# robertknight/ocrs

Measured on AMD Instinct MI355X. Metric: pages/sec end-to-end (1024x1024), higher is better.
Workload: dtype f32

## Files before the change

### include/ocrs_amd.h

```cpp
#ifndef OCRS_AMD_H
#define OCRS_AMD_H

#include <stddef.h>
#include <stdint.h>

#if defined(__GNUC__)
#define OCRS_API __attribute__((visibility("default")))
#else
#define OCRS_API
#endif

#ifdef __cplusplus
extern "C" {
#endif

typedef enum ocrs_status {
    OCRS_OK = 0,
    OCRS_ERR_INVALID_ARGUMENT = 1,
    OCRS_ERR_MODEL_NOT_LOADED = 2,
    OCRS_ERR_MODEL_DIMS = 3,
    OCRS_ERR_RUN_FAILED = 4,
    OCRS_ERR_WRONG_OUTPUT = 5,
    OCRS_ERR_IMAGE_SOURCE = 6,
    OCRS_ERR_DEVICE = 7,
// ... 23 lines not shown

OCRS_API ocrs_status ocrs_mask_component_rects(const uint8_t* masks, size_t n, int h, int w, float expand, float min_area,
                                               int max_comp, int64_t arena, int32_t* n_roots, int32_t* overflow, float* rects,
                                               uint8_t* valid);

OCRS_API ocrs_status ocrs_gru_tile_plan(const int32_t* lengths_desc, size_t n_lines, int hidden, int32_t* n_clusters, int32_t* waves,
                                        int16_t* tiles);

OCRS_API ocrs_status ocrs_coalescer_selftest(int n_threads, int requests_per_thread, int max_active, int max_pages,
                                             long window_us, int fail_every, uint64_t out[5]);

OCRS_API ocrs_status ocrs_stream_plan_selftest(int budget, const int32_t* ops, size_t n_ops, int32_t* out);

OCRS_API ocrs_status ocrs_conv_rows_selftest(const float* w, size_t n_w, const float* bias, size_t n_bias, int relu, int y0, int h,
                                             int cin, int32_t out[6]);

OCRS_API ocrs_status ocrs_set_option(const char* name, long value);
OCRS_API ocrs_status ocrs_option_name(int index, const char** name);

OCRS_API ocrs_status ocrs_device_pool_stats(int device, uint64_t out[12]);
OCRS_API ocrs_status ocrs_device_pool_configure(int device, uint64_t device_cached_cap_bytes, uint64_t pinned_cached_cap_bytes);
OCRS_API ocrs_status ocrs_device_pool_trim(int device);

typedef enum { OCRS_ISOLATION_AUTO = 0, OCRS_ISOLATION_NONE = 1 } ocrs_isolation;
OCRS_API ocrs_status ocrs_device_set_isolation(int device, ocrs_isolation policy);
OCRS_API ocrs_status ocrs_device_isolation(int device, int out[3]);

typedef struct ocrs_model ocrs_model;

OCRS_API ocrs_status ocrs_model_load_file(const char* path, ocrs_model** out);
// ... 428 lines not shown
```

### ocrs_amd/_lib.py

```python
import ctypes as C
import os

_HERE = os.path.dirname(os.path.abspath(__file__))
LIB_PATH = os.environ.get("OCRS_AMD_LIB") or os.path.join(_HERE, "libocrs_amd.so")

OCRS_OK = 0
STATUS_NAMES = {
    0: "OK", 1: "INVALID_ARGUMENT", 2: "MODEL_NOT_LOADED", 3: "MODEL_DIMS", 4: "RUN_FAILED", 5: "WRONG_OUTPUT",
    6: "IMAGE_SOURCE", 7: "DEVICE", 8: "IO", 9: "CAPACITY",
}

RUN_FN = C.CFUNCTYPE(C.c_int, C.c_void_p, C.POINTER(C.c_float), C.POINTER(C.c_int64), C.POINTER(C.POINTER(C.c_float)),
                     C.POINTER(C.c_int64), C.POINTER(C.c_int))


class EngineParams(C.Structure):
    _fields_ = [("detection_model", C.c_void_p), ("recognition_model", C.c_void_p), ("debug", C.c_int),
                ("decode_method", C.c_int), ("beam_width", C.c_uint32), ("alphabet", C.c_char_p),
                ("allowed_chars", C.c_char_p), ("numerics", C.c_int), ("coalesce", C.c_int), ("coalesce_pages", C.c_int),
                ("coalesce_window_us", C.c_int), ("layout_threads", C.c_int), ("rec_max_pixels", C.c_int64)]


class GroupParams(C.Structure):
    _fields_ = [("detection_model", C.c_void_p), ("detection_model_len", C.c_size_t), ("recognition_model", C.c_void_p),
# ... 24 lines not shown
    "ocrs_last_error", "ocrs_buffer_free", "ocrs_device_count", "ocrs_set_device", "ocrs_set_option", "ocrs_ctc_beam_search", "ocrs_model_load_file",
    "ocrs_model_load_bytes", "ocrs_model_from_callback", "ocrs_model_input_shape", "ocrs_model_run",
    "ocrs_model_flops", "ocrs_model_free", "ocrs_engine_new", "ocrs_engine_free", "ocrs_image_source_check_bytes",
    "ocrs_engine_prepare_input", "ocrs_engine_prepare_input_device", "ocrs_page_free", "ocrs_page_dims",
    "ocrs_page_image", "ocrs_engine_detect_words", "ocrs_engine_detect_words_batch",
    "ocrs_engine_detect_text_pixels", "ocrs_engine_detection_threshold", "ocrs_engine_find_text_lines",
    "ocrs_engine_find_text_lines_batch",
    "ocrs_engine_recognize_text", "ocrs_engine_recognize_text_batch", "ocrs_engine_recognize_tokens",
    "ocrs_engine_prepare_recognition_input", "ocrs_text_item_rotated_rect", "ocrs_rotated_rect_corners", "ocrs_engine_get_text", "ocrs_device_malloc", "ocrs_device_free",
    "ocrs_device_upload", "ocrs_device_synchronize", "ocrs_device_measure_peaks", "ocrs_engine_enable_timing", "ocrs_stage_count",
    "ocrs_stage_name", "ocrs_engine_stage_times", "ocrs_kernel_class_count", "ocrs_kernel_class_name",
    "ocrs_engine_kernel_stats", "ocrs_engine_set_kernel_timing_mask", "ocrs_gru_tile_plan", "ocrs_host_malloc", "ocrs_host_free", "ocrs_engine_prepare_input_batch",
    "ocrs_get_device", "ocrs_model_load_file_on_device", "ocrs_model_load_bytes_on_device", "ocrs_model_device", "ocrs_engine_device",
    "ocrs_engine_group_new", "ocrs_engine_group_free", "ocrs_engine_group_size", "ocrs_engine_group_member", "ocrs_group_deal",
    "ocrs_group_prepare_input_batch", "ocrs_group_prepare_input_device_batch", "ocrs_group_detect_words_batch",
    "ocrs_group_recognize_text_batch", "ocrs_group_gather", "ocrs_group_final_gather", "ocrs_group_worker_threads", "ocrs_group_last_gather", "ocrs_device_malloc_on", "ocrs_engine_coalesce_stats", "ocrs_coalescer_selftest", "ocrs_stream_plan_selftest", "ocrs_conv_rows_selftest", "ocrs_engine_kernel_mfma_flops", "ocrs_engine_prepare_input_jpeg", "ocrs_jpeg_decode_rgb", "ocrs_jpeg_info", "ocrs_jpeg_coefficients",
    "ocrs_group_member_stats", "ocrs_numa_parse_cpulist", "ocrs_numa_bind_selftest", "ocrs_engine_recognize_logits", "ocrs_engine_set_option", "ocrs_engine_get_option", "ocrs_option_name", "ocrs_device_pool_stats", "ocrs_device_pool_configure", "ocrs_device_pool_trim",
    "ocrs_device_set_isolation", "ocrs_device_isolation", "ocrs_group_set_replay", "ocrs_abi_version",
    "ocrs_engine_recognize_text_scored", "ocrs_engine_recognize_text_batch_scored", "ocrs_ctc_beam_search_scored",
    "ocrs_engine_run_recognition_ops", "ocrs_ctc_decode_packed", "ocrs_mask_component_rects",
    "ocrs_engine_detect_words_scored", "ocrs_engine_detect_words_batch_scored", "ocrs_group_detect_words_batch_scored",
    "ocrs_engine_find_text_lines_indexed", "ocrs_engine_find_text_lines_batch_indexed",
    "ocrs_detection_tile_plan", "ocrs_engine_detect_words_tiled", "ocrs_engine_detect_words_batch_tiled",
    "ocrs_engine_detect_text_pixels_tiled", "ocrs_group_detect_words_batch_tiled",
    "ocrs_line_frame", "ocrs_line_char_boxes", "ocrs_engine_prepare_recognition_input_rectified",
    "ocrs_engine_recognize_text_rectified", "ocrs_engine_recognize_text_batch_rectified",
    "ocrs_group_recognize_text_batch_rectified", "ocrs_engine_recognize_tokens_rectified",
    "ocrs_engine_rotate_page", "ocrs_engine_rotate_pages", "ocrs_unrotate_rects", "ocrs_unrotate_chars",
    "ocrs_orientation_vote", "ocrs_engine_detect_orientation", "ocrs_engine_page_from_grey",
    "ocrs_engine_resize_page", "ocrs_engine_resize_pages", "ocrs_work_size", "ocrs_rescale_rects",
    "ocrs_engine_detect_words_at", "ocrs_engine_detect_words_batch_at",
# ... 303 lines not shown
```

### ocrs_amd/csrc/abi.cpp

```cpp
#include <cstdio>
#include <fstream>
#include <thread>

#include <atomic>
#include "abi_util.hpp"
#include "coalesce_selftest.hpp"
#include "conv_rows.hpp"
#include "engine.hpp"
#include "host_pool.hpp"
#include "jpeg.hpp"
#include "kernels.hpp"
#include "page_ops.hpp"

using namespace ocrs;
using namespace ocrs::geom;

using namespace ocrs::abi;

extern "C" {

const char* ocrs_last_error(void) { return last_error().c_str(); }

void ocrs_buffer_free(void* p) { free(p); }

// ... 61 lines not shown

ocrs_status ocrs_conv_rows_selftest(const float* w, size_t n_w, const float* bias, size_t n_bias, int relu, int y0, int h, int cin,
                                    int32_t out[6]) {
    return guarded([&] {
        if (!out || (n_w > 0 && !w) || (n_bias > 0 && !bias) || h < kConvRowsPatchH || h % kConvRowsPatchH != 0 || y0 < 0 || y0 >= h ||
            y0 % kConvRowsPatchH != 0 || cin < 2 * kConvRowsChunk || cin % (2 * kConvRowsChunk) != 0)
            fail(OCRS_ERR_INVALID_ARGUMENT, "bad argument");
        out[0] = conv_rows_skip_exact(w, n_w, bias, n_bias, relu != 0) ? 1 : 0;
        const RowPhases ph = conv_row_phases(y0, h, cin, out[0] != 0);
        out[1] = ph.c_top;
        out[2] = ph.c_bot;
        for (int phase = 0; phase < 3; phase++) {
            const int c = 3 * phase * (cin / kConvRowsChunk);
            out[3 + phase] = c < ph.c_top ? 0 : c >= ph.c_bot ? kConvRowsPatchH - 1 : -1;
        }
    });
}

namespace {

void beam_search_hook(const float* logp, int t, int c, uint32_t width, int impl, std::vector<uint32_t>* l,
                      std::vector<uint32_t>* p, double* score, std::vector<float>* step_logp) {
    if (impl == 2 && t > 0) {
        DeviceScope bind(-1);
        if (!k::ctc_beam_supported(c, (int)width)) fail(OCRS_ERR_CAPACITY, "beam search on the GPU supports up to 128 classes and width 128");
        Workspace ws;
        std::vector<int32_t> meta(1 + t + 1);
        meta[0] = t;
        for (int i = 0; i <= t; i++) meta[1 + i] = i;
        int32_t* d_meta = ws.alloc_n<int32_t>(meta.size());
// ... 1066 lines not shown
```

### ocrs_amd/csrc/common.cpp

```cpp
#include "common.hpp"

#include <chrono>
#include <climits>
#include <cstdint>
#include <cstdlib>
#include <cstring>

#include <algorithm>
#include <atomic>
#include <condition_variable>
#include <deque>
#include <system_error>

namespace ocrs {

static thread_local std::string g_last_error;

void set_last_error(const std::string& msg) { g_last_error = msg; }
const std::string& last_error() { return g_last_error; }

namespace {
std::atomic<int> g_default_device{0};
thread_local DeviceContext* t_ctx = nullptr;
constexpr int kMaxDevices = 64;
// ... 430 lines not shown
const OptRange kOptRanges[OPT_COUNT] = {
    {0, 1, {}}, {0, 1, {}}, {0, 1, {}}, {0, 2, {}}, {0, 1, {8, 14, 32}}, {0, 1, {8, 14, 20, 32}}, {0, 1, {}}, {0, 1, {}}, {0, 1, {}}, {0, 1, {}},
    {1, 1024, {}}, {LanePlan::kMinBudget, LanePlan::kMaxBudget, {}},
    {0, 2, {}}, {0, 64, {}}, {1, 4096, {}}, {0, 10000000, {}}, {0, 4096, {}}, {0, INT64_MAX, {}},
};
bool in_range(int i, long v) {
    const OptRange& r = kOptRanges[i];
    if (i == OPT_STREAM_BUDGET) return LanePlan::valid_budget(v);
    if (v >= r.lo && v <= r.hi) return true;
    for (long a : r.also) if (a && v == a) return true;
    return false;
}
const char* const kRetired[] = {"det_heavy", "det_tail", "gru_waves", "gru_background", "gru_scatter", "gru_gates_pack", "conv_occupancy",
                                "gx_heavy", "gemm_nfast", "conv_a_lds", "gru_heavy", "heavy_priority", "det_mfma"};
std::atomic<long> g_opts[OPT_COUNT];
std::once_flag g_opts_once;
void init_options() {
    for (int i = 0; i < OPT_COUNT; i++) {
        const char* e = kOptDefs[i].env ? getenv(kOptDefs[i].env) : nullptr;
        const long v = e && *e ? strtol(e, nullptr, 10) : kOptDefs[i].def;
        g_opts[i].store(in_range(i, v) ? v : kOptDefs[i].def);
    }
}
int find_option(const char* name, int count = OPT_PUBLIC_COUNT) {
    for (int i = 0; i < count; i++)
        if (name && i != OPT_NUMERICS && strcmp(name, kOptDefs[i].name) == 0) return i;
    return -1;
}
thread_local const Tuning* t_tuning = nullptr;
}
// ... 2 lines not shown
TuningScope::~TuningScope() { t_tuning = prev_; }
const Tuning* current_tuning() { return t_tuning; }

long process_option(Option o) {
    std::call_once(g_opts_once, init_options);
    return g_opts[o].load(std::memory_order_relaxed);
}

long option_long(Option o) {
    if (t_tuning) return __atomic_load_n(&t_tuning->v[o], __ATOMIC_RELAXED);
    std::call_once(g_opts_once, init_options);
    return g_opts[o].load(std::memory_order_relaxed);
}
int option(Option o) { return (int)option_long(o); }
int conv_rows_setting() { return t_tuning ? (int)__atomic_load_n(&t_tuning->conv_rows, __ATOMIC_RELAXED) : (int)kConvRowsDefault; }

Tuning default_tuning() {
    std::call_once(g_opts_once, init_options);
    Tuning t;
    for (int i = 0; i < OPT_COUNT; i++) t.v[i] = g_opts[i].load(std::memory_order_relaxed);
    t.conv_rows = kConvRowsDefault;
    return t;
}

const char* option_name(int i) { return i >= 0 && i < OPT_PUBLIC_COUNT ? kOptDefs[i].name : nullptr; }

int set_option(const char* name, long value) {
    std::call_once(g_opts_once, init_options);
    const int i = find_option(name);
    if (i < 0) {
        for (const char* r : kRetired) if (name && strcmp(name, r) == 0) return 0;
        return 1;
    }
    if (!in_range(i, value)) return 2;
    if (i == OPT_STREAM_BUDGET && value != g_opts[i].load() && any_device_has_calls_in_flight()) return 3;
    g_opts[i].store(value);
    return 0;
}

int set_option(Tuning& t, const char* name, long value) {
    if (name && strcmp(name, "conv_rows") == 0) {
        if (value < 0 || value > 2) return 2;
        __atomic_store_n(&t.conv_rows, value, __ATOMIC_RELAXED);
        return 0;
    }
    const int i = find_option(name, OPT_COUNT);
    if (i < 0) return 1;
    if (i == OPT_STREAM_BUDGET) return 4;
    if (!in_range(i, value)) return 2;
    __atomic_store_n(&t.v[i], value, __ATOMIC_RELAXED);
    return 0;
}

bool get_option(const Tuning& t, const char* name, long* value) {
    if (name && strcmp(name, "conv_rows") == 0) {
        *value = __atomic_load_n(&t.conv_rows, __ATOMIC_RELAXED);
        return true;
    }
    const int i = name && strcmp(name, "numerics") == 0 ? (int)OPT_NUMERICS : find_option(name, OPT_COUNT);
    if (i < 0) return false;
    *value = __atomic_load_n(&t.v[i], __ATOMIC_RELAXED);
    return true;
}

static hipEvent_t take_lease_event(DeviceContext* c) {
    {
        std::lock_guard<std::mutex> g(c->stream_mu);
        if (!c->lease_events.empty()) {
            hipEvent_t e = c->lease_events.back();
            c->lease_events.pop_back();
            return e;
// ... 139 lines not shown
```

### ocrs_amd/csrc/common.hpp

```cpp
#pragma once
#include <atomic>
#include <hip/hip_runtime.h>

#include <cstdarg>
#include <cstdint>
#include <cstdio>
#include <cstdlib>
#include <chrono>
#include <condition_variable>
#include <cstring>
#include <map>
#include <mutex>
#include <stdexcept>
#include <string>
#include <thread>
#include <vector>

#include "../../include/ocrs_amd.h"
#include "stream_plan.hpp"

namespace ocrs {

struct Error : std::runtime_error {
    ocrs_status status;
// ... 116 lines not shown
    DeviceContext* prev_;
    int restore_ = -1;
};

inline DevicePool& pool() { return ctx().pool; }
inline HostPool& host_pool() { return ctx().host_pool; }
inline hipStream_t heavy_stream() { return ctx().heavy_stream(); }

enum Option { OPT_GRU_MODE = 0, OPT_GRU_GATES, OPT_GRU_LOCAL, OPT_DET_FUSE, OPT_DET_STREAM, OPT_DET_ROWS, OPT_CCL_QUAD,
              OPT_CONV12_FUSE, OPT_CONV_FLAT, OPT_BEAM_GPU, OPT_DET_TILE_BATCH, OPT_STREAM_BUDGET, OPT_PUBLIC_COUNT,
              OPT_NUMERICS = OPT_PUBLIC_COUNT,
              OPT_COALESCE, OPT_COALESCE_PAGES, OPT_COALESCE_WINDOW_US,
              OPT_LAYOUT_THREADS, OPT_REC_MAX_PIXELS,
              OPT_COUNT };
constexpr long kConvRowsDefault = 2;
struct Tuning { long v[OPT_COUNT]; long conv_rows; };
int conv_rows_setting();
Tuning default_tuning();
int set_option(const char* name, long value);
int set_option(Tuning& t, const char* name, long value);
bool get_option(const Tuning& t, const char* name, long* value);
const char* option_name(int i);
class TuningScope {
  public:
    explicit TuningScope(const Tuning* t);
    ~TuningScope();
    TuningScope(const TuningScope&) = delete;
    TuningScope& operator=(const TuningScope&) = delete;
  private:
    const Tuning* prev_;
};
const Tuning* current_tuning();
// ... 204 lines not shown
```

### ocrs_amd/csrc/conv_rows.hpp

```cpp
#pragma once
#include <cmath>
#include <cstddef>
#include <cstring>

namespace ocrs {

constexpr int kConvRowsChunk = 16;
constexpr int kConvRowsPatchH = 4;

inline bool conv_rows_skip_exact(const float* w, size_t n_w, const float* bias, size_t n_bias, bool relu) {
    for (size_t i = 0; i < n_w; i++)
        if (!std::isfinite(w[i])) return false;
    if (relu) return true;
    for (size_t i = 0; i < n_bias; i++) {
        unsigned u;
        memcpy(&u, &bias[i], 4);
        if (u == 0x80000000u) return false;
    }
    return true;
}

struct RowPhases { int c_top, c_bot; };
constexpr RowPhases conv_row_phases(int y0, int H, int cin, bool skip) {
    const int per_tap = cin / kConvRowsChunk;
// ... 5 lines not shown
```

### ocrs_amd/csrc/kernels.hpp

```cpp
#pragma once
#include <vector>
#include <hip/hip_runtime.h>

#include <cstdint>

namespace ocrs {
namespace jpeg { struct Coefficients; }
namespace k {

void prepare_image(const void* d_pixels, bool is_u8, bool chans_last, int h, int w, int chans, float* d_out,
                   hipStream_t s);
struct PrepareTable {
    enum { kPages = 32 };
    const void* src[kPages];
    float* dst[kPages];
};
void prepare_image_batch(const void* const* d_pixels, float* const* d_out, int n, bool is_u8, bool chans_last, int h, int w,
                         int chans, hipStream_t s);
void resize_pages_to_model(const float* const* d_src_ptrs, int n, int sh, int sw, int vh, int vw, float* d_dst,
                           int dh, int dw, hipStream_t s);
bool resize_threshold(const float* d_prob, int n, int mh, int mw, int sh, int sw, float thr, uint8_t* d_mask,
                      float* d_map, int h, int w, hipStream_t s, int32_t* d_labels = nullptr, int32_t* d_zero_a = nullptr,
                      int32_t* d_zero_b = nullptr);
void threshold_only(const float* d_prob, float thr, uint8_t* d_mask, int64_t count, hipStream_t s);
// ... 68 lines not shown
    float* y;
    float* ypool;
    int n, h, w, h1, w1;
    int relu_d1, relu_p1, relu_d2, relu_p2, sigmoid;
    int tiles_x, tiles_y;
    const float* tape = nullptr;
    int tape_len = 0;
    const float* rtape = nullptr;
    int rtape_len = 0;
};
struct StreamWeights {
    const float *wt, *bt, *wd1, *bd1, *wp1, *bp1, *wd2, *bd2, *wp2, *bp2, *wf, *bf;
};
bool double_conv_fused(const DoubleConvArgs& a, int cs, int cx, int cmid, int cout, bool pool, bool final_conv,
                       bool launch, hipStream_t s, bool* on_mfma = nullptr, int* path = nullptr);
bool double_conv_stream(const DoubleConvArgs& a, int cs, int cx, int cmid, int cout, bool pool, bool final_conv, bool launch, hipStream_t s,
                        const StreamWeights* hw = nullptr, std::vector<float>* tape_out = nullptr, int* tape_len = nullptr);
bool double_conv_rows(const DoubleConvArgs& a, int cs, int cx, int cmid, int cout, bool pool, bool final_conv, bool launch, hipStream_t s,
                      const StreamWeights* hw = nullptr, std::vector<float>* tape_out = nullptr, int* tape_len = nullptr);
bool double_conv_rows_takes(const DoubleConvArgs& a, int cx);
void maxpool(const float* x, int n, int h, int w, int c, int kh, int kw, float* y, hipStream_t s);
void avgpool(const float* x, int n, int h, int w, int c, int kh, int kw, float* y, hipStream_t s);
void padcat(const float* skip, int n, int sh, int sw, int cs, const float* x, int h, int w, int cx, float* y,
            hipStream_t s);
void sigmoid(const float* x, float* y, int64_t count, hipStream_t s);
void conv1x1_cout1(const float* x, int64_t pixels, int cin, const float* wt, const float* bias, int relu, int do_sigmoid,
                   float* y, hipStream_t s);
void to_seq(const float* x, int n, int w, int c, float* y, hipStream_t s);
void gru_gates(const float* gx, const float* gh, float* h, float* y, int T, int N, int H, int step, hipStream_t s);
bool log_softmax_argmax(const float* logits, int64_t rows, int c, const uint8_t* d_excluded ,
// ... 283 lines not shown
```

### ocrs_amd/csrc/kernels_det.hip

```cpp
#include "common.hpp"
#include "kernels.hpp"
#include "spec_math.hpp"

namespace ocrs {
namespace k {

namespace {

typedef float f32x4 __attribute__((ext_vector_type(4)));

__device__ __forceinline__ int floor_div2(int v) { return v >> 1; }

template <int CS_, int CX_, int CMID_, int COUT_, int TH_, int TW_, bool POOL_, bool FINAL_>
struct McCfg {
    static constexpr int NT = 512;
    static constexpr int CS = CS_, CX = CX_, CMID = CMID_, COUT = COUT_, TH = TH_, TW = TW_;
    static constexpr bool POOL = POOL_, FINAL = FINAL_, DEC = CX_ > 0;
    static constexpr int CU = DEC ? CS_ : 0;
    static constexpr int CIN = CS + CU;
    static constexpr bool ONE = CIN == 1;
    static constexpr int P = TW_ >= 32 ? 4 : 2;
    static constexpr int SA = ONE ? 1 : CIN + 4, SD1 = ONE ? 1 : CIN + 4, SC = CMID + 4, SD2 = CMID + 4, SE = COUT + 4, SX = CX + 4;
    static constexpr int R0H = TH + 4, R0W = TW + 4, R1H = TH + 2, R1W = TW + 2;
    static constexpr int LH = (TH + 4) / 2 + 1, LW = (TW + 4) / 2 + 1;
    static constexpr int NPIX0 = R0H * R0W, NPIX1 = R1H * R1W, NPIX2 = TH * TW;
    static constexpr int A_FLOATS = NPIX0 * SA, C_FLOATS = NPIX1 * SC;
    static constexpr int X_FLOATS = DEC ? LH * LW * SX : 0, D1_FLOATS = ONE ? 0 : NPIX1 * SD1, D2_FLOATS = NPIX2 * SD2;
    static constexpr int E_FLOATS = POOL ? NPIX2 * SE : 0;
    static constexpr int max3(int x, int y, int z) { return (x > y ? x : y) > z ? (x > y ? x : y) : z; }
    static constexpr int U_RAW = ONE ? max3(A_FLOATS, D2_FLOATS, 0) : max3(A_FLOATS, C_FLOATS, E_FLOATS);
    static constexpr int V_RAW = ONE ? max3(C_FLOATS, E_FLOATS, 0) : max3(X_FLOATS, D1_FLOATS, D2_FLOATS);
    static constexpr int U_FLOATS = (U_RAW + 3) / 4 * 4 + 64, V_FLOATS = (V_RAW + 3) / 4 * 4 + 64;
    static constexpr int W_FLOATS = 10 * CIN + 10 * CMID;
    static constexpr size_t LDS_BYTES = (size_t)(U_FLOATS + V_FLOATS + W_FLOATS) * sizeof(float);
};

template <int K> __device__ __forceinline__ constexpr int ch_pos(int c) { return (c & 3) * (K / 4) + (c >> 2); }
template <int K> __device__ __forceinline__ constexpr int ch_of(int n) { return (n % (K / 4)) * 4 + n / (K / 4); }

template <int K, int P, int S_IN, int S_OUT>
__device__ __forceinline__ void dw_stage(const float* __restrict__ src, int srcw, float* __restrict__ dst, int rows, int cols,
                                         const float* __restrict__ sw, bool relu, int tid, int nt) {
    constexpr int NB = K / 4;
    const int ns = (cols + P - 1) / P;
    const int items = rows * ns * NB;
    for (int it = tid; it < items; it += nt) {
        const int blk = it % NB;
        const int t2 = it / NB;
        const int strip = t2 % ns, r = t2 / ns;
        const int x0 = strip * P;
        f32x4 acc[P];
        const f32x4 bias = *reinterpret_cast<const f32x4*>(sw + 9 * K + 4 * blk);
#pragma unroll
        for (int j = 0; j < P; j++) acc[j] = bias;
#pragma unroll
        for (int dy = 0; dy < 3; dy++) {
            f32x4 row[P + 2];
#pragma unroll
            for (int j = 0; j < P + 2; j++) {
                const int xx = x0 + j < srcw ? x0 + j : srcw - 1;
                row[j] = *reinterpret_cast<const f32x4*>(src + ((r + dy) * srcw + xx) * S_IN + 4 * blk);
            }
#pragma unroll
            for (int dx = 0; dx < 3; dx++) {
                const f32x4 wv = *reinterpret_cast<const f32x4*>(sw + (dy * 3 + dx) * K + 4 * blk);
#pragma unroll
                for (int j = 0; j < P; j++) {
#pragma unroll
                    for (int e = 0; e < 4; e++) acc[j][e] = fmaf(row[j + dx][e], wv[e], acc[j][e]);
                }
            }
        }
#pragma unroll
        for (int j = 0; j < P; j++) {
            if (x0 + j < cols) {
                f32x4 v = acc[j];
// ... 12 lines not shown
    if constexpr (KS == 1) {
        b[0] = p[0];
    } else if constexpr (KS == 2) {
        const float2 v = *reinterpret_cast<const float2*>(p);
        b[0] = v.x; b[1] = v.y;
    } else {
#pragma unroll
        for (int q = 0; q < KS / 4; q++) {
            const f32x4 v = *reinterpret_cast<const f32x4*>(p + 4 * q);
            b[4 * q] = v[0]; b[4 * q + 1] = v[1]; b[4 * q + 2] = v[2]; b[4 * q + 3] = v[3];
        }
    }
}

template <class Cfg>
__global__ void __launch_bounds__(Cfg::NT)
double_conv_mfma_kernel(DoubleConvArgs a) {
    constexpr int NT = Cfg::NT, NW = Cfg::NT / 64;
    constexpr int CS = Cfg::CS, CX = Cfg::CX, CU = Cfg::CU, CIN = Cfg::CIN, CMID = Cfg::CMID, COUT = Cfg::COUT;
    constexpr int TH = Cfg::TH, TW = Cfg::TW, SA = Cfg::SA, SD1 = Cfg::SD1, SC = Cfg::SC, SD2 = Cfg::SD2, SE = Cfg::SE, SX = Cfg::SX;
    constexpr int R0H = Cfg::R0H, R0W = Cfg::R0W, R1H = Cfg::R1H, R1W = Cfg::R1W, LH = Cfg::LH, LW = Cfg::LW;
    constexpr int NPIX0 = Cfg::NPIX0, NPIX1 = Cfg::NPIX1, NPIX2 = Cfg::NPIX2, P = Cfg::P;
    extern __shared__ __attribute__((aligned(16))) float lds[];
    float* sU = lds;
    float* sV = lds + Cfg::U_FLOATS;
    float* sW1 = sV + Cfg::V_FLOATS;
    float* sW2 = sW1 + 10 * CIN;
    const int tid = threadIdx.x;
    const int lane = tid & 63, wave = tid >> 6;
    const int i16 = lane & 15, kq = lane >> 4;
    const int nblk = gridDim.x;
// ... 13 lines not shown
    for (int i = tid; i < 10 * CMID; i += NT) {
        const int t = i / CMID, n = i - t * CMID;
        const int c = ch_of<CMID>(n);
        sW2[i] = t < 9 ? a.wd2[t * CMID + c] : a.bd2[c];
    }

    float* sA = sU;
    const float* __restrict__ skip = a.skip + (int64_t)img * h * w * CS;
    if constexpr (Cfg::ONE) {
        for (int p = tid; p < NPIX0; p += NT) {
            const int gy = Y0 - 2 + p / R0W, gx = X0 - 2 + p % R0W;
            float v = 0.f;
            if ((unsigned)gy < (unsigned)h && (unsigned)gx < (unsigned)w) v = skip[(int64_t)gy * w + gx];
            sA[p] = v;
        }
    } else {
        constexpr int Q = CS / 4;
        for (int i = tid; i < NPIX0 * Q; i += NT) {
            const int p = i / Q, c4 = i - p * Q;
            const int gy = Y0 - 2 + p / R0W, gx = X0 - 2 + p % R0W;
            f32x4 v = {0.f, 0.f, 0.f, 0.f};
            if ((unsigned)gy < (unsigned)h && (unsigned)gx < (unsigned)w)
                v = *reinterpret_cast<const f32x4*>(skip + ((int64_t)gy * w + gx) * CS + c4 * 4);
#pragma unroll
            for (int e = 0; e < 4; e++) sA[p * SA + ch_pos<CIN>(c4 * 4 + e)] = v[e];
        }
    }
    if constexpr (Cfg::DEC) {
        float* sX = sV;
        const int pyo = (h - 2 * a.h1) / 2, pxo = (w - 2 * a.w1) / 2;
        const int ly0 = floor_div2(Y0 - 2 - pyo), lx0 = floor_div2(X0 - 2 - pxo);
        const float* __restrict__ x1 = a.x1 + (int64_t)img * a.h1 * a.w1 * CX;
        constexpr int QX = CX / 4, NLOW = LH * LW;
        for (int i = tid; i < NLOW * QX; i += NT) {
            const int p = i / QX, c4 = i - p * QX;
            const int ly = ly0 + p / LW, lx = lx0 + p % LW;
            f32x4 v = {0.f, 0.f, 0.f, 0.f};
            if ((unsigned)ly < (unsigned)a.h1 && (unsigned)lx < (unsigned)a.w1)
                v = *reinterpret_cast<const f32x4*>(x1 + ((int64_t)ly * a.w1 + lx) * CX + c4 * 4);
#pragma unroll
            for (int e = 0; e < 4; e++) sX[p * SX + ch_pos<CX>(c4 * 4 + e)] = v[e];
        }
        for (int i = tid; i < NPIX0 * CU; i += NT) {
            const int p = i / CU, c = i - p * CU;
            sA[p * SA + ch_pos<CIN>(CS + c)] = 0.f;
        }
        constexpr int KSX = CX / 4, NGT = (4 * CU) / 16;
        float at[NGT][KSX];
        f32x4 biast[NGT];
#pragma unroll
        for (int g = 0; g < NGT; g++) {
            const int n = 16 * g + i16, q = n / CU, co = n % CU;
#pragma unroll
            for (int s4 = 0; s4 < KSX; s4++) at[g][s4] = a.wt[((size_t)q * CX + 4 * s4 + kq) * CU + co];
#pragma unroll
            for (int r = 0; r < 4; r++) biast[g][r] = a.bt[(16 * g + 4 * kq + r) % CU];
        }
        __syncthreads();
        for (int pg = wave; pg * 16 < NLOW; pg += NW) {
            const int p = pg * 16 + i16;
            const int pc = p < NLOW ? p : NLOW - 1;
            float b[KSX];
            load_b<KSX>(sX + pc * SX + kq * KSX, b);
            const int ly = ly0 + pc / LW, lx = lx0 + pc % LW;
            const bool src_ok = p < NLOW && (unsigned)ly < (unsigned)a.h1 && (unsigned)lx < (unsigned)a.w1;
#pragma unroll
            for (int g = 0; g < NGT; g++) {
                f32x4 acc = biast[g];
#pragma unroll
                for (int s4 = 0; s4 < KSX; s4++) acc = __builtin_amdgcn_mfma_f32_16x16x4f32(at[g][s4], b[s4], acc, 0, 0, 0);
                const int n0 = 16 * g + 4 * kq;
                const int q = n0 / CU, co0 = n0 % CU;
                const int gy = 2 * ly + (q >> 1) + pyo, gx = 2 * lx + (q & 1) + pxo;
                const int ry = gy - (Y0 - 2), rx = gx - (X0 - 2);
                if (src_ok && (unsigned)ry < (unsigned)R0H && (unsigned)rx < (unsigned)R0W && (unsigned)gy < (unsigned)h &&
                    (unsigned)gx < (unsigned)w) {
#pragma unroll
                    for (int r = 0; r < 4; r++) sA[(ry * R0W + rx) * SA + ch_pos<CIN>(CS + co0 + r)] = acc[r];
                }
            }
        }
    }
    __syncthreads();

    float* sC = sU;
    if constexpr (Cfg::ONE) {
        float* sCt = sV;
        for (int p = tid; p < NPIX1; p += NT) {
            const int ry = p / R1W, rx = p - ry * R1W;
            const int gy = Y0 - 1 + ry, gx = X0 - 1 + rx;
            float* dst = &sCt[p * SC];
            if ((unsigned)gy >= (unsigned)h || (unsigned)gx >= (unsigned)w) {
#pragma unroll
// ... 3 lines not shown
            float d = sW1[9];
#pragma unroll
            for (int t = 0; t < 9; t++) d = fmaf(sA[(ry + t / 3) * R0W + rx + t % 3], sW1[t], d);
            if (a.relu_d1) d = d > 0.f ? d : 0.f;
#pragma unroll
            for (int c = 0; c < CMID; c++) {
                float o = fmaf(d, a.wp1[c], a.bp1[c]);
                if (a.relu_p1) o = o > 0.f ? o : 0.f;
                dst[ch_pos<CMID>(c)] = o;
            }
        }
        __syncthreads();
        sC = sCt;
    } else {
        float* sD1 = sV;
        dw_stage<CIN, P, SA, SD1>(sA, R0W, sD1, R1H, R1W, sW1, a.relu_d1 != 0, tid, NT);
        constexpr int KS = CIN / 4, NG = (CMID + 15) / 16;
        float aw[NG][KS];
        f32x4 bias1[NG];
#pragma unroll
        for (int g = 0; g < NG; g++) {
            const int n = 16 * g + i16;
            const int co = n < CMID ? ch_of<CMID>(n) : 0;
#pragma unroll
            for (int s4 = 0; s4 < KS; s4++) aw[g][s4] = n < CMID ? a.wp1[(4 * s4 + kq) * CMID + co] : 0.f;
#pragma unroll
            for (int r = 0; r < 4; r++) {
                const int nr = 16 * g + 4 * kq + r;
                bias1[g][r] = nr < CMID ? a.bp1[ch_of<CMID>(nr)] : 0.f;
            }
        }
// ... 123 lines not shown

bool double_conv_fused(const DoubleConvArgs& a, int cs, int cx, int cmid, int cout, bool pool, bool final_conv,
                       bool launch, hipStream_t s, bool* on_mfma, int* path) {
    if (path) *path = 0;
    if (option(OPT_DET_ROWS) >= 1 && ((!launch && a.n == 0) || a.rtape) && double_conv_rows_takes(a, cx) &&
        double_conv_rows(a, cs, cx, cmid, cout, pool, final_conv, launch, s)) {
        if (on_mfma) *on_mfma = true;
        if (path) *path = 2;
        return true;
    }
    if (option(OPT_DET_STREAM) >= 1 && ((!launch && a.n == 0) || a.tape) && double_conv_stream(a, cs, cx, cmid, cout, pool, final_conv, launch, s)) {
        if (on_mfma) *on_mfma = false;
        if (path) *path = 1;
        return true;
    }
#define OCRS_DC(CS, CX, CM, CO, TH, TW, P, F)                                                   \
    if (cs == CS && cx == CX && cmid == CM && cout == CO && pool == P && final_conv == F) {      \
        if (on_mfma) *on_mfma = true;                                                            \
        if (launch) launch_mc<McCfg<CS, CX, CM, CO, TH, TW, P, F>>(a, s);                        \
        return true;                                                                             \
    }
    OCRS_DC(1, 0, 8, 8, 16, 32, true, false)
    OCRS_DC(8, 0, 16, 16, 8, 32, true, false)
    OCRS_DC(16, 0, 32, 32, 8, 16, true, false)
    OCRS_DC(32, 0, 32, 32, 8, 16, true, false)
    OCRS_DC(8, 16, 8, 8, 8, 32, false, true)
    OCRS_DC(8, 16, 8, 8, 8, 32, false, false)
    OCRS_DC(16, 32, 16, 16, 8, 16, false, false)
    OCRS_DC(32, 32, 32, 32, 8, 16, false, false)
    OCRS_DC(32, 64, 32, 32, 8, 16, false, false)
#undef OCRS_DC
    return false;
}

}
}
```

### ocrs_amd/csrc/kernels_rec.hip

```cpp
#include <algorithm>
#include <type_traits>

#include "common.hpp"
#include "conv_rows.hpp"
#include "kernels.hpp"
#include "split_mfma.hpp"

namespace ocrs {
namespace k {

typedef float f32x16 __attribute__((ext_vector_type(16)));
typedef unsigned u32x4 __attribute__((ext_vector_type(4)));
typedef float f32x4 __attribute__((ext_vector_type(4)));
typedef float f32x2 __attribute__((ext_vector_type(2)));
typedef unsigned u32x2 __attribute__((ext_vector_type(2)));
typedef __bf16 bf16x8 __attribute__((ext_vector_type(8)));
typedef __bf16 bf16x2 __attribute__((ext_vector_type(2)));

__device__ __forceinline__ int xcd_remap(int b, int nwg) {
    const int xcd = b & 7, q = nwg >> 3, r = nwg & 7;
    return (xcd < r ? xcd * (q + 1) : r * (q + 1) + (xcd - r) * q) + (b >> 3);
}

__device__ __forceinline__ int find_group(const int32_t* __restrict__ toff, int G, int tile) {
// ... 184 lines not shown
void avgpool_to_seq_ragged(const float* x, const RaggedView& in, const RaggedView& seq, int c, const int32_t* d_pos,
                           const int32_t* d_off, float* y, hipStream_t s) {
    if (seq.ntiles256 <= 0) return;
    hipLaunchKernelGGL(avgpool_to_seq_ragged_kernel, dim3(seq.ntiles256), dim3(256), 0, s, x, in, seq, c, d_pos, d_off, y);
}

void to_seq_packed_ragged(const float* x, const RaggedView& in, int c, const int32_t* d_pos, const int32_t* d_off,
                          float* y, hipStream_t s) {
    if (in.ntiles256 <= 0) return;
    hipLaunchKernelGGL(to_seq_packed_ragged_kernel, dim3(in.ntiles256), dim3(256), 0, s, x, in, c, d_pos, d_off, y);
}

constexpr int RG_BM = 128, RG_BK = 16, RG_LDA = RG_BM + 1;
constexpr int CONV_WAVES = 4;
static_assert(RG_BK == kConvRowsChunk && RG_BM / 32 == kConvRowsPatchH, "conv_rows.hpp describes this kernel's K loop");
template <int BN, int TW, int PH, int PW, int ROWS, bool FLAT, int SPLIT = 0>
__global__ void __launch_bounds__(256, SPLIT == 3 ? 2 : SPLIT == 2 ? 3 : CONV_WAVES)
conv3x3_ragged_kernel(const float* __restrict__ X, RaggedView rv, int cin, const float* __restrict__ Bw,
                      const float* __restrict__ bias, int cout, int relu, float* __restrict__ Y,
                      const int64_t* __restrict__ out_poff, int skip) {
    extern __shared__ __attribute__((aligned(16))) float lds[];
    constexpr int NTW = BN / 64;
    constexpr int TH = RG_BM / TW;
    static_assert(TW == 32 || TW == 16, "patch width");
    static_assert(!ROWS || (SPLIT == 0 && BN == 128 && TW == 32), "row-owning waves: exact, 128 columns, 4 x 32 patches");
    static_assert(!SPLIT || (BN == 128 && RG_BK == 16), "split mode: 128-column blocks, 16-deep chunks");
    constexpr int NP = SPLIT ? SPLIT : 1;
    constexpr int SP_PLANE = split::PLANE;
    float* As = lds;
    float* Bs = lds + (SPLIT ? 2 * NP * SP_PLANE : 2 * RG_BK * RG_LDA);
// ... 805 lines not shown
        rv.toff2d_flat = rv_in.toff2d_flat_32; rv.ntiles2d_flat = rv_in.ntiles2d_flat_32;
        rv.toff2d_flat2 = rv_in.toff2d_flat2_32; rv.ntiles2d_flat2 = rv_in.ntiles2d_flat2_32;
        rv.max_tile_px_ = rv_in.max_tile_px32_;
    }
    if (rv.tw != 32 && rv.tw != 16) return false;
    if (rv.H % (RG_BM / rv.tw) != 0) return false;
    const bool flat = option(OPT_CONV_FLAT) != 0 && rv.min_w >= 11 &&
                      rv.max_tile_px_ * std::max(cin, cout) * (int64_t)sizeof(float) < (int64_t)1 << 30;
    if (!flat && (int64_t)rv.H * rv.max_w * cin * (int64_t)sizeof(float) >= (int64_t)1 << 30) return false;
    const int ntiles = flat ? (pw == 2 ? rv.ntiles2d_flat2 : rv.ntiles2d_flat) : rv.ntiles2d;
    if (ntiles <= 0) return true;
    const bool n64 = cout <= 64;
    const int numerics = option(OPT_NUMERICS);
    const bool split = wsplit && !n64 && (cout % 128) == 0 && (cin % 64) == 0 && numerics != 0;
    const size_t lds = split ? split::lds_bytes(numerics == 2 ? 2 : 3)
                             : (size_t)(2 * RG_BK * RG_LDA + 2 * RG_BK * (n64 ? 64 : 128)) * sizeof(float);
    const dim3 grid(ntiles, (cout + (n64 ? 63 : 127)) / (n64 ? 64 : 128));
#define OCRS_LAUNCH_SPLIT(TW_, PH_, PW_, FLAT_, NP_, SLOT_)                                                              \
    if (flat == FLAT_ && (numerics == 2 ? 2 : 3) == NP_) {                                                              \
        allow_dynamic_lds(reinterpret_cast<const void*>(&conv3x3_ragged_kernel<128, TW_, PH_, PW_, 0, FLAT_, NP_>), ok_[SLOT_]);   \
        hipLaunchKernelGGL((conv3x3_ragged_kernel<128, TW_, PH_, PW_, 0, FLAT_, NP_>), grid, dim3(256), lds, s, x, rv, cin, ws_, bias, \
                           cout, relu, y, out.poff, 0);                                                                 \
    }
#define OCRS_LAUNCH_CONV(BN_, TW_, PH_, PW_)                                                                            \
    do {                                                                                                                \
        if (split && BN_ == 128) {                                                                                      \
            const float* ws_ = reinterpret_cast<const float*>(wsplit);                                                  \
            static std::atomic<uint64_t> ok_[4] = {};                                                                    \
            OCRS_LAUNCH_SPLIT(TW_, PH_, PW_, true, 3, 0) OCRS_LAUNCH_SPLIT(TW_, PH_, PW_, false, 3, 1)                     \
            OCRS_LAUNCH_SPLIT(TW_, PH_, PW_, true, 2, 2) OCRS_LAUNCH_SPLIT(TW_, PH_, PW_, false, 2, 3)                     \
        } else if (flat) hipLaunchKernelGGL((conv3x3_ragged_kernel<BN_, TW_, PH_, PW_, 0, true>), grid, dim3(256), lds, s, x, rv, \
// ... 36 lines not shown
```

Before: 288.1.

## Add lean 256-thread detection double-conv variants sized to co-reside with conv blocks

Adds a 'lean' configuration of the fused detection double-conv MFMA kernel that uses 256 threads, smaller tiles, and a two-phase staged load of skip and upsampled channels. Its LDS footprint is capped so it fits beside three resident ragged-conv blocks, so detection can overlap with recognition convs on the same CU. Upsample weights are reloaded per group instead of held in registers when they would be too large. The variant is on by default for batches larger than 8 and can be selected through a new det_lean option. It trades per-block throughput for higher occupancy and co-residency.

Result: no change. 287.5 (-0.2%).

```diff
diff --git a/include/ocrs_amd.h b/include/ocrs_amd.h
--- a/include/ocrs_amd.h
+++ b/include/ocrs_amd.h
@@ -61,6 +61,9 @@
 
 OCRS_API ocrs_status ocrs_conv_rows_selftest(const float* w, size_t n_w, const float* bias, size_t n_bias, int relu, int y0, int h,
                                              int cin, int32_t out[6]);
+
+OCRS_API ocrs_status ocrs_det_block_query(int cs, int cx, int cmid, int cout, int pool, int final_conv, int n, int h, int w,
+                                          int h1, int w1, int tapes, int32_t out[3]);
 
 OCRS_API ocrs_status ocrs_set_option(const char* name, long value);
 OCRS_API ocrs_status ocrs_option_name(int index, const char** name);
diff --git a/ocrs_amd/_lib.py b/ocrs_amd/_lib.py
--- a/ocrs_amd/_lib.py
+++ b/ocrs_amd/_lib.py
@@ -62,7 +62,7 @@
     "ocrs_get_device", "ocrs_model_load_file_on_device", "ocrs_model_load_bytes_on_device", "ocrs_model_device", "ocrs_engine_device",
     "ocrs_engine_group_new", "ocrs_engine_group_free", "ocrs_engine_group_size", "ocrs_engine_group_member", "ocrs_group_deal",
     "ocrs_group_prepare_input_batch", "ocrs_group_prepare_input_device_batch", "ocrs_group_detect_words_batch",
-    "ocrs_group_recognize_text_batch", "ocrs_group_gather", "ocrs_group_final_gather", "ocrs_group_worker_threads", "ocrs_group_last_gather", "ocrs_device_malloc_on", "ocrs_engine_coalesce_stats", "ocrs_coalescer_selftest", "ocrs_stream_plan_selftest", "ocrs_conv_rows_selftest", "ocrs_engine_kernel_mfma_flops", "ocrs_engine_prepare_input_jpeg", "ocrs_jpeg_decode_rgb", "ocrs_jpeg_info", "ocrs_jpeg_coefficients",
+    "ocrs_group_recognize_text_batch", "ocrs_group_gather", "ocrs_group_final_gather", "ocrs_group_worker_threads", "ocrs_group_last_gather", "ocrs_device_malloc_on", "ocrs_engine_coalesce_stats", "ocrs_coalescer_selftest", "ocrs_stream_plan_selftest", "ocrs_conv_rows_selftest", "ocrs_det_block_query","ocrs_engine_kernel_mfma_flops", "ocrs_engine_prepare_input_jpeg", "ocrs_jpeg_decode_rgb", "ocrs_jpeg_info", "ocrs_jpeg_coefficients",
     "ocrs_group_member_stats", "ocrs_numa_parse_cpulist", "ocrs_numa_bind_selftest", "ocrs_engine_recognize_logits", "ocrs_engine_set_option", "ocrs_engine_get_option", "ocrs_option_name", "ocrs_device_pool_stats", "ocrs_device_pool_configure", "ocrs_device_pool_trim",
     "ocrs_device_set_isolation", "ocrs_device_isolation", "ocrs_group_set_replay", "ocrs_abi_version",
     "ocrs_engine_recognize_text_scored", "ocrs_engine_recognize_text_batch_scored", "ocrs_ctc_beam_search_scored",
diff --git a/ocrs_amd/csrc/abi.cpp b/ocrs_amd/csrc/abi.cpp
--- a/ocrs_amd/csrc/abi.cpp
+++ b/ocrs_amd/csrc/abi.cpp
@@ -99,6 +99,22 @@
             const int c = 3 * phase * (cin / kConvRowsChunk);
             out[3 + phase] = c < ph.c_top ? 0 : c >= ph.c_bot ? kConvRowsPatchH - 1 : -1;
         }
+    });
+}
+
+ocrs_status ocrs_det_block_query(int cs, int cx, int cmid, int cout, int pool, int final_conv, int n, int h, int w, int h1, int w1,
+                                 int tapes, int32_t out[3]) {
+    return guarded([&] {
+        if (!out || n < 0 || h < 1 || w < 1 || h1 < 0 || w1 < 0) fail(OCRS_ERR_INVALID_ARGUMENT, "bad argument");
+        static const float dummy = 0.f;
+        k::DoubleConvArgs a{};
+        a.n = n; a.h = h; a.w = w; a.h1 = h1; a.w1 = w1;
+        if (tapes) { a.tape = &dummy; a.rtape = &dummy; }
+        bool on_mfma = false;
+        int path = 0;
+        out[0] = k::double_conv_fused(a, cs, cx, cmid, cout, pool != 0, final_conv != 0, false, nullptr, &on_mfma, &path) ? 1 : 0;
+        out[1] = out[0] ? path : -1;
+        out[2] = det_lean_setting();
     });
 }
 
diff --git a/ocrs_amd/csrc/common.cpp b/ocrs_amd/csrc/common.cpp
--- a/ocrs_amd/csrc/common.cpp
+++ b/ocrs_amd/csrc/common.cpp
@@ -468,6 +468,8 @@
 const char* const kRetired[] = {"det_heavy", "det_tail", "gru_waves", "gru_background", "gru_scatter", "gru_gates_pack", "conv_occupancy",
                                 "gx_heavy", "gemm_nfast", "conv_a_lds", "gru_heavy", "heavy_priority", "det_mfma"};
 std::atomic<long> g_opts[OPT_COUNT];
+std::atomic<long> g_det_lean{kDetLeanDefault};
+bool is_det_lean(const char* name) { return name && strcmp(name, "det_lean") == 0; }
 std::once_flag g_opts_once;
 void init_options() {
     for (int i = 0; i < OPT_COUNT; i++) {
@@ -500,12 +502,16 @@
 }
 int option(Option o) { return (int)option_long(o); }
 int conv_rows_setting() { return t_tuning ? (int)__atomic_load_n(&t_tuning->conv_rows, __ATOMIC_RELAXED) : (int)kConvRowsDefault; }
+int det_lean_setting() {
+    return (int)(t_tuning ? __atomic_load_n(&t_tuning->det_lean, __ATOMIC_RELAXED) : g_det_lean.load(std::memory_order_relaxed));
+}
 
 Tuning default_tuning() {
     std::call_once(g_opts_once, init_options);
     Tuning t;
     for (int i = 0; i < OPT_COUNT; i++) t.v[i] = g_opts[i].load(std::memory_order_relaxed);
     t.conv_rows = kConvRowsDefault;
+    t.det_lean = g_det_lean.load(std::memory_order_relaxed);
     return t;
 }
 
@@ -513,6 +519,11 @@
 
 int set_option(const char* name, long value) {
     std::call_once(g_opts_once, init_options);
+    if (is_det_lean(name)) {
+        if (value < 0 || value > 2) return 2;
+        g_det_lean.store(value);
+        return 0;
+    }
     const int i = find_option(name);
     if (i < 0) {
         for (const char* r : kRetired) if (name && strcmp(name, r) == 0) return 0;
@@ -528,6 +539,11 @@
     if (name && strcmp(name, "conv_rows") == 0) {
         if (value < 0 || value > 2) return 2;
         __atomic_store_n(&t.conv_rows, value, __ATOMIC_RELAXED);
+        return 0;
+    }
+    if (is_det_lean(name)) {
+        if (value < 0 || value > 2) return 2;
+        __atomic_store_n(&t.det_lean, value, __ATOMIC_RELAXED);
         return 0;
     }
     const int i = find_option(name, OPT_COUNT);
@@ -541,6 +557,10 @@
 bool get_option(const Tuning& t, const char* name, long* value) {
     if (name && strcmp(name, "conv_rows") == 0) {
         *value = __atomic_load_n(&t.conv_rows, __ATOMIC_RELAXED);
+        return true;
+    }
+    if (is_det_lean(name)) {
+        *value = __atomic_load_n(&t.det_lean, __ATOMIC_RELAXED);
         return true;
     }
     const int i = name && strcmp(name, "numerics") == 0 ? (int)OPT_NUMERICS : find_option(name, OPT_COUNT);
diff --git a/ocrs_amd/csrc/common.hpp b/ocrs_amd/csrc/common.hpp
--- a/ocrs_amd/csrc/common.hpp
+++ b/ocrs_amd/csrc/common.hpp
@@ -154,8 +154,10 @@
               OPT_LAYOUT_THREADS, OPT_REC_MAX_PIXELS,
               OPT_COUNT };
 constexpr long kConvRowsDefault = 2;
-struct Tuning { long v[OPT_COUNT]; long conv_rows; };
+constexpr long kDetLeanDefault = 1;
+struct Tuning { long v[OPT_COUNT]; long conv_rows; long det_lean; };
 int conv_rows_setting();
+int det_lean_setting();
 Tuning default_tuning();
 int set_option(const char* name, long value);
 int set_option(Tuning& t, const char* name, long value);
diff --git a/ocrs_amd/csrc/conv_rows.hpp b/ocrs_amd/csrc/conv_rows.hpp
--- a/ocrs_amd/csrc/conv_rows.hpp
+++ b/ocrs_amd/csrc/conv_rows.hpp
@@ -7,6 +7,7 @@
 
 constexpr int kConvRowsChunk = 16;
 constexpr int kConvRowsPatchH = 4;
+constexpr size_t kConvRaggedLdsBytes = (size_t)(2 * kConvRowsChunk * (128 + 1) + 2 * kConvRowsChunk * 128) * sizeof(float);
 
 inline bool conv_rows_skip_exact(const float* w, size_t n_w, const float* bias, size_t n_bias, bool relu) {
     for (size_t i = 0; i < n_w; i++)
diff --git a/ocrs_amd/csrc/kernels.hpp b/ocrs_amd/csrc/kernels.hpp
--- a/ocrs_amd/csrc/kernels.hpp
+++ b/ocrs_amd/csrc/kernels.hpp
@@ -106,6 +106,7 @@
 };
 bool double_conv_fused(const DoubleConvArgs& a, int cs, int cx, int cmid, int cout, bool pool, bool final_conv,
                        bool launch, hipStream_t s, bool* on_mfma = nullptr, int* path = nullptr);
+constexpr bool double_conv_lean_takes(int n) { return n > 8; }
 bool double_conv_stream(const DoubleConvArgs& a, int cs, int cx, int cmid, int cout, bool pool, bool final_conv, bool launch, hipStream_t s,
                         const StreamWeights* hw = nullptr, std::vector<float>* tape_out = nullptr, int* tape_len = nullptr);
 bool double_conv_rows(const DoubleConvArgs& a, int cs, int cx, int cmid, int cout, bool pool, bool final_conv, bool launch, hipStream_t s,
diff --git a/ocrs_amd/csrc/kernels_det.hip b/ocrs_amd/csrc/kernels_det.hip
--- a/ocrs_amd/csrc/kernels_det.hip
+++ b/ocrs_amd/csrc/kernels_det.hip
@@ -1,4 +1,5 @@
 #include "common.hpp"
+#include "conv_rows.hpp"
 #include "kernels.hpp"
 #include "spec_math.hpp"
 
@@ -11,16 +12,24 @@
 
 __device__ __forceinline__ int floor_div2(int v) { return v >> 1; }
 
-template <int CS_, int CX_, int CMID_, int COUT_, int TH_, int TW_, bool POOL_, bool FINAL_>
+constexpr size_t kLeanLdsBudget = 160 * 1024 - 3 * kConvRaggedLdsBytes;
+constexpr size_t kLeanLdsAim = 56 * 1024;
+
+template <int CS_, int CX_, int CMID_, int COUT_, int TH_, int TW_, bool POOL_, bool FINAL_, int NT_ = 512, int G_ = 1>
 struct McCfg {
-    static constexpr int NT = 512;
+    static constexpr int NT = NT_;
+    static constexpr bool LEAN = NT_ == 256;
+    static constexpr int G = G_;
     static constexpr int CS = CS_, CX = CX_, CMID = CMID_, COUT = COUT_, TH = TH_, TW = TW_;
     static constexpr bool POOL = POOL_, FINAL = FINAL_, DEC = CX_ > 0;
     static constexpr int CU = DEC ? CS_ : 0;
     static constexpr int CIN = CS + CU;
     static constexpr bool ONE = CIN == 1;
     static constexpr int P = TW_ >= 32 ? 4 : 2;
-    static constexpr int SA = ONE ? 1 : CIN + 4, SD1 = ONE ? 1 : CIN + 4, SC = CMID + 4, SD2 = CMID + 4, SE = COUT + 4, SX = CX + 4;
+    static constexpr int SA = ONE ? 1 : CIN / G + 4, SD1 = ONE ? 1 : CIN + 4, SC = CMID + 4, SD2 = CMID + 4, SE = COUT + 4, SX = CX + 4;
+    static_assert(NT_ == 512 || NT_ == 256, "");
+    static_assert(G_ == 1 || (G_ == 2 && DEC && CU == CS_ && CIN % 32 == 0), "staging: one group is the skip half, the other the upsampled half");
+    static_assert((TH_ * TW_) % 16 == 0 && TH_ % 2 == 0 && TW_ % 2 == 0, "");
     static constexpr int R0H = TH + 4, R0W = TW + 4, R1H = TH + 2, R1W = TW + 2;
     static constexpr int LH = (TH + 4) / 2 + 1, LW = (TW + 4) / 2 + 1;
     static constexpr int NPIX0 = R0H * R0W, NPIX1 = R1H * R1W, NPIX2 = TH * TW;
@@ -33,19 +42,24 @@
     static constexpr int U_FLOATS = (U_RAW + 3) / 4 * 4 + 64, V_FLOATS = (V_RAW + 3) / 4 * 4 + 64;
     static constexpr int W_FLOATS = 10 * CIN + 10 * CMID;
     static constexpr size_t LDS_BYTES = (size_t)(U_FLOATS + V_FLOATS + W_FLOATS) * sizeof(float);
+    static_assert(!LEAN || LDS_BYTES <= kLeanLdsBudget, "a lean block fits beside three resident conv blocks");
+    static_assert(!LEAN || LDS_BYTES <= kLeanLdsAim, "... with headroom");
 };
 
 template <int K> __device__ __forceinline__ constexpr int ch_pos(int c) { return (c & 3) * (K / 4) + (c >> 2); }
 template <int K> __device__ __forceinline__ constexpr int ch_of(int n) { return (n % (K / 4)) * 4 + n / (K / 4); }
 
-template <int K, int P, int S_IN, int S_OUT>
+template <int K, int P, int S_IN, int S_OUT, int G = 1>
 __device__ __forceinline__ void dw_stage(const float* __restrict__ src, int srcw, float* __restrict__ dst, int rows, int cols,
-                                         const float* __restrict__ sw, bool relu, int tid, int nt) {
-    constexpr int NB = K / 4;
+                                         const float* __restrict__ sw, bool relu, int tid, int nt, int grp = 0) {
+    constexpr int NB = K / 4 / G;
+    constexpr int KB = K / 16 > 0 ? K / 16 : 1, KG = KB / G > 0 ? KB / G : 1;
+    static_assert(G == 1 || (G == 2 && K % 32 == 0), "");
     const int ns = (cols + P - 1) / P;
     const int items = rows * ns * NB;
     for (int it = tid; it < items; it += nt) {
-        const int blk = it % NB;
+        const int lb = it % NB;
+        const int blk = G == 1 ? lb : (lb / KG) * KB + grp * KG + lb % KG;
         const int t2 = it / NB;
         const int strip = t2 % ns, r = t2 / ns;
         const int x0 = strip * P;
@@ -59,7 +73,7 @@
 #pragma unroll
             for (int j = 0; j < P + 2; j++) {
                 const int xx = x0 + j < srcw ? x0 + j : srcw - 1;
-                row[j] = *reinterpret_cast<const f32x4*>(src + ((r + dy) * srcw + xx) * S_IN + 4 * blk);
+                row[j] = *reinterpret_cast<const f32x4*>(src + ((r + dy) * srcw + xx) * S_IN + 4 * lb);
             }
 #pragma unroll
             for (int dx = 0; dx < 3; dx++) {
@@ -102,7 +116,7 @@
 }
 
 template <class Cfg>
-__global__ void __launch_bounds__(Cfg::NT)
+__global__ void __launch_bounds__(Cfg::NT, Cfg::LEAN ? 4 : 2)
 double_conv_mfma_kernel(DoubleConvArgs a) {
     constexpr int NT = Cfg::NT, NW = Cfg::NT / 64;
     constexpr int CS = Cfg::CS, CX = Cfg::CX, CU = Cfg::CU, CIN = Cfg::CIN, CMID = Cfg::CMID, COUT = Cfg::COUT;
@@ -146,8 +160,11 @@
             if ((unsigned)gy < (unsigned)h && (unsigned)gx < (unsigned)w) v = skip[(int64_t)gy * w + gx];
             sA[p] = v;
         }
-    } else {
-        constexpr int Q = CS / 4;
+    }
+    constexpr bool STAGED = Cfg::G == 2;
+    constexpr int CA = STAGED ? CS : CIN;
+    auto load_skip = [&]() {
+        constexpr int Q = Cfg::ONE ? 1 : CS / 4;
         for (int i = tid; i < NPIX0 * Q; i += NT) {
             const int p = i / Q, c4 = i - p * Q;
             const int gy = Y0 - 2 + p / R0W, gx = X0 - 2 + p % R0W;
@@ -155,10 +172,12 @@
             if ((unsigned)gy < (unsigned)h && (unsigned)gx < (unsigned)w)
                 v = *reinterpret_cast<const f32x4*>(skip + ((int64_t)gy * w + gx) * CS + c4 * 4);
 #pragma unroll
-            for (int e = 0; e < 4; e++) sA[p * SA + ch_pos<CIN>(c4 * 4 + e)] = v[e];
-        }
-    }
+            for (int e = 0; e < 4; e++) sA[p * SA + ch_pos<Cfg::ONE ? 4 : CA>(c4 * 4 + e)] = v[e];
+        }
+    };
+    if constexpr (!Cfg::ONE && !STAGED) load_skip();
     if constexpr (Cfg::DEC) {
+        constexpr int UP0 = STAGED ? 0 : CS;
         float* sX = sV;
         const int pyo = (h - 2 * a.h1) / 2, pxo = (w - 2 * a.w1) / 2;
         const int ly0 = floor_div2(Y0 - 2 - pyo), lx0 = floor_div2(X0 - 2 - pxo);
@@ -175,18 +194,23 @@
         }
         for (int i = tid; i < NPIX0 * CU; i += NT) {
             const int p = i / CU, c = i - p * CU;
-            sA[p * SA + ch_pos<CIN>(CS + c)] = 0.f;
+            sA[p * SA + ch_pos<CA>(UP0 + c)] = 0.f;
         }
         constexpr int KSX = CX / 4, NGT = (4 * CU) / 16;
-        float at[NGT][KSX];
-        f32x4 biast[NGT];
-#pragma unroll
-        for (int g = 0; g < NGT; g++) {
+        constexpr bool AT_REGS = !Cfg::LEAN || NGT * KSX <= 32;
+        constexpr int NAT = AT_REGS ? NGT : 1;
+        float at[NAT][KSX];
+        f32x4 biast[NAT];
+        auto load_at = [&](int g, float (&ag)[KSX], f32x4& bg) {
             const int n = 16 * g + i16, q = n / CU, co = n % CU;
 #pragma unroll
-            for (int s4 = 0; s4 < KSX; s4++) at[g][s4] = a.wt[((size_t)q * CX + 4 * s4 + kq) * CU + co];
-#pragma unroll
-            for (int r = 0; r < 4; r++) biast[g][r] = a.bt[(16 * g + 4 * kq + r) % CU];
+            for (int s4 = 0; s4 < KSX; s4++) ag[s4] = a.wt[((size_t)q * CX + 4 * s4 + kq) * CU + co];
+#pragma unroll
+            for (int r = 0; r < 4; r++) bg[r] = a.bt[(16 * g + 4 * kq + r) % CU];
+        };
+        if constexpr (AT_REGS) {
+#pragma unroll
+            for (int g = 0; g < NGT; g++) load_at(g, at[g], biast[g]);
         }
         __syncthreads();
         for (int pg = wave; pg * 16 < NLOW; pg += NW) {
@@ -198,9 +222,11 @@
             const bool src_ok = p < NLOW && (unsigned)ly < (unsigned)a.h1 && (unsigned)lx < (unsigned)a.w1;
 #pragma unroll
             for (int g = 0; g < NGT; g++) {
-                f32x4 acc = biast[g];
-#pragma unroll
-                for (int s4 = 0; s4 < KSX; s4++) acc = __builtin_amdgcn_mfma_f32_16x16x4f32(at[g][s4], b[s4], acc, 0, 0, 0);
+                constexpr int GI = AT_REGS ? 1 : 0;
+                if constexpr (!AT_REGS) load_at(g, at[0], biast[0]);
+                f32x4 acc = biast[g * GI];
+#pragma unroll
+                for (int s4 = 0; s4 < KSX; s4++) acc = __builtin_amdgcn_mfma_f32_16x16x4f32(at[g * GI][s4], b[s4], acc, 0, 0, 0);
                 const int n0 = 16 * g + 4 * kq;
                 const int q = n0 / CU, co0 = n0 % CU;
                 const int gy = 2 * ly + (q >> 1) + pyo, gx = 2 * lx + (q & 1) + pxo;
@@ -208,7 +234,7 @@
                 if (src_ok && (unsigned)ry < (unsigned)R0H && (unsigned)rx < (unsigned)R0W && (unsigned)gy < (unsigned)h &&
                     (unsigned)gx < (unsigned)w) {
 #pragma unroll
-                    for (int r = 0; r < 4; r++) sA[(ry * R0W + rx) * SA + ch_pos<CIN>(CS + co0 + r)] = acc[r];
+                    for (int r = 0; r < 4; r++) sA[(ry * R0W + rx) * SA + ch_pos<CA>(UP0 + co0 + r)] = acc[r];
                 }
             }
         }
@@ -242,7 +268,15 @@
         sC = sCt;
     } else {
         float* sD1 = sV;
-        dw_stage<CIN, P, SA, SD1>(sA, R0W, sD1, R1H, R1W, sW1, a.relu_d1 != 0, tid, NT);
+        if constexpr (STAGED) {
+            dw_stage<CIN, P, SA, SD1, 2>(sA, R0W, sD1, R1H, R1W, sW1, a.relu_d1 != 0, tid, NT, 1);
+            __syncthreads();
+            load_skip();
+            __syncthreads();
+            dw_stage<CIN, P, SA, SD1, 2>(sA, R0W, sD1, R1H, R1W, sW1, a.relu_d1 != 0, tid, NT, 0);
+        } else {
+            dw_stage<CIN, P, SA, SD1>(sA, R0W, sD1, R1H, R1W, sW1, a.relu_d1 != 0, tid, NT);
+        }
         constexpr int KS = CIN / 4, NG = (CMID + 15) / 16;
         float aw[NG][KS];
         f32x4 bias1[NG];
@@ -396,6 +430,16 @@
         if (path) *path = 1;
         return true;
     }
+    const int lean_opt = det_lean_setting();
+    const bool lean = lean_opt == 2 || (lean_opt == 1 && double_conv_lean_takes(a.n));
+#define OCRS_DC_LEAN(CS, CX, CM, CO, TH, TW, P, F, LTH, LTW, G)                                 \
+    if (lean && cs == CS && cx == CX && cmid == CM && cout == CO && pool == P && final_conv == F) { \
+        if (on_mfma) *on_mfma = true;                                                            \
+        if (path) *path = 3;                                                                     \
+        if (launch) launch_mc<McCfg<CS, CX, CM, CO, LTH, LTW, P, F, 256, G>>(a, s);              \
+        return true;                                                                             \
+    }                                                                                            \
+    OCRS_DC(CS, CX, CM, CO, TH, TW, P, F)
 #define OCRS_DC(CS, CX, CM, CO, TH, TW, P, F)                                                   \
     if (cs == CS && cx == CX && cmid == CM && cout == CO && pool == P && final_conv == F) {      \
         if (on_mfma) *on_mfma = true;                                                            \
@@ -403,14 +447,15 @@
         return true;                                                                             \
     }
     OCRS_DC(1, 0, 8, 8, 16, 32, true, false)
-    OCRS_DC(8, 0, 16, 16, 8, 32, true, false)
-    OCRS_DC(16, 0, 32, 32, 8, 16, true, false)
-    OCRS_DC(32, 0, 32, 32, 8, 16, true, false)
+    OCRS_DC_LEAN(8, 0, 16, 16, 8, 32, true, false, 8, 32, 1)
+    OCRS_DC_LEAN(16, 0, 32, 32, 8, 16, true, false, 8, 16, 1)
+    OCRS_DC_LEAN(32, 0, 32, 32, 8, 16, true, false, 8, 8, 1)
     OCRS_DC(8, 16, 8, 8, 8, 32, false, true)
     OCRS_DC(8, 16, 8, 8, 8, 32, false, false)
-    OCRS_DC(16, 32, 16, 16, 8, 16, false, false)
-    OCRS_DC(32, 32, 32, 32, 8, 16, false, false)
-    OCRS_DC(32, 64, 32, 32, 8, 16, false, false)
+    OCRS_DC_LEAN(16, 32, 16, 16, 8, 16, false, false, 8, 8, 1)
+    OCRS_DC_LEAN(32, 32, 32, 32, 8, 16, false, false, 8, 8, 2)
+    OCRS_DC_LEAN(32, 64, 32, 32, 8, 16, false, false, 8, 8, 2)
+#undef OCRS_DC_LEAN
 #undef OCRS_DC
     return false;
 }
diff --git a/ocrs_amd/csrc/kernels_rec.hip b/ocrs_amd/csrc/kernels_rec.hip
--- a/ocrs_amd/csrc/kernels_rec.hip
+++ b/ocrs_amd/csrc/kernels_rec.hip
@@ -222,6 +222,7 @@
 constexpr int RG_BM = 128, RG_BK = 16, RG_LDA = RG_BM + 1;
 constexpr int CONV_WAVES = 4;
 static_assert(RG_BK == kConvRowsChunk && RG_BM / 32 == kConvRowsPatchH, "conv_rows.hpp describes this kernel's K loop");
+static_assert(kConvRaggedLdsBytes == (size_t)(2 * RG_BK * RG_LDA + 2 * RG_BK * 128) * sizeof(float), "... and its 128-column block's LDS");
 template <int BN, int TW, int PH, int PW, int ROWS, bool FLAT, int SPLIT = 0>
 __global__ void __launch_bounds__(256, SPLIT == 3 ? 2 : SPLIT == 2 ? 3 : CONV_WAVES)
 conv3x3_ragged_kernel(const float* __restrict__ X, RaggedView rv, int cin, const float* __restrict__ Bw,
@@ -1057,7 +1058,7 @@
     const int numerics = option(OPT_NUMERICS);
     const bool split = wsplit && !n64 && (cout % 128) == 0 && (cin % 64) == 0 && numerics != 0;
     const size_t lds = split ? split::lds_bytes(numerics == 2 ? 2 : 3)
-                             : (size_t)(2 * RG_BK * RG_LDA + 2 * RG_BK * (n64 ? 64 : 128)) * sizeof(float);
+                             : n64 ? (size_t)(2 * RG_BK * RG_LDA + 2 * RG_BK * 64) * sizeof(float) : kConvRaggedLdsBytes;
     const dim3 grid(ntiles, (cout + (n64 ? 63 : 127)) / (n64 ? 64 : 128));
 #define OCRS_LAUNCH_SPLIT(TW_, PH_, PW_, FLAT_, NP_, SLOT_)                                                              \
     if (flat == FLAT_ && (numerics == 2 ? 2 : 3) == NP_) {                                                              \
```
